# MengRao/pollnet

Hardware: AMD Instinct MI355X
Metric: device-resident Gbit/s + Mframes/s, 1500 B IPv4/TCP frames, 1/2/4/8 MI355X (higher is better)
Workload: dtype u16/u32 integer (one's-complement sums)

## Files before the change

### pollnet_amd/csrc/frame_pass.hpp

```cpp
#pragma once

#include <type_traits>

#include "device_common.hpp"

namespace pn_dev {

constexpr int kWave = 64;
constexpr int kFramesPerWave = 64;
constexpr int kBatch = 8;
constexpr int kLoadAux = 2;
constexpr int kStoreAux = 16;

constexpr int kWinChunks = 7;
constexpr int kWinBytes = 16 * kWinChunks;
using Window = Win<4 * kWinChunks>;

constexpr uint32_t kPadUnknown = 0xFFFFFFFFu;

enum : int { kAblNoProbe = 1, kAblNoReduce = 2 };
enum : int { kExactRange = 64 };
enum : int { kCoopProbe = 256 };
enum : int { kSkipEmptyLoads = 1024 };
enum : int { kSkipWaveGate = 16384 };
// ... 293 lines not shown
    }
#pragma unroll
    for (int j = 0; j < kBatch; ++j) {
      const int end = ends[j], s0 = s0s[j];
      if (end > s0 + 2048) {
        const __amdgpu_buffer_rsrc_t rs = frame_rsrc(frame_win(b0 + j), (uint32_t)(end + 15) & ~15u);
        uint32_t sum = acc[j];
        for (int kb = s0 + 2048; kb < end; kb += 1024) {
          const u32x4 w = __builtin_amdgcn_raw_buffer_load_b128(rs, kb + lane * 16, 0, LAUX);
          const int o = kb + lane * 16;
          sum = dot2(w.x, tail_sel(end, o), sum);
          sum = dot2(w.y, tail_sel(end, o + 4), sum);
          sum = dot2(w.z, tail_sel(end, o + 8), sum);
          sum = dot2(w.w, tail_sel(end, o + 12), sum);
        }
        acc[j] = sum;
      }
    }
    if constexpr (ABL & kAblNoReduce) {
      uint32_t x = 0;
#pragma unroll
      for (int j = 0; j < kBatch; ++j) x += acc[j];
      if ((uint32_t)(lane >> 3) == b0 / kBatch) t_all += x;
    } else {
#pragma unroll
      for (int i = 0; i < 4; ++i) {
        const auto r = __builtin_amdgcn_permlane32_swap(acc[i], acc[i + 4], false, false);
        acc[i] = r[0] + r[1];
      }
#pragma unroll
      for (int i = 0; i < 2; ++i) {
        const auto r = __builtin_amdgcn_permlane16_swap(acc[i], acc[i + 2], false, false);
        acc[i] = r[0] + r[1];
      }
      const bool b3 = lane & 8;
      const uint32_t keep = b3 ? acc[1] : acc[0];
      const uint32_t send = b3 ? acc[0] : acc[1];
      uint32_t v = keep + dpp<0x128>(send);
      v += dpp<0xB1>(v);
      v += dpp<0x4E>(v);
      v += dpp<0x141>(v);
      const uint32_t tot = __shfl(v, (lane & 7) * 8);
      if ((uint32_t)(lane >> 3) == b0 / kBatch) t_all += tot;
    }
  }
}

template <int ABL, int LAUX, int IDX>
__device__ __forceinline__ void stream_phase_pipelined(uint32_t stride, const uint8_t* group_ipa, uint64_t my_win,
                                                       uint32_t n_here, int lane, int end_rel, uint32_t& t_all,
                                                       uint32_t& pad) {
  static_assert(!(ABL & kSkipEmptyLoads) && (ABL & kExactRange), "pipelined phase 2: every load issued, exact ranges");
  constexpr int kHalf = kBatch / 2;
  auto frame_win = [&](uint32_t fi) -> const uint8_t* {
    if constexpr (IDX) {
      const uint32_t lo = __builtin_amdgcn_readlane((uint32_t)my_win, fi & 63);
      const uint32_t hi = __builtin_amdgcn_readlane((uint32_t)(my_win >> 32), fi & 63);
      return (const uint8_t*)(((uint64_t)hi << 32) | lo);
    } else {
      return group_ipa + (uint64_t)fi * stride;
    }
  };
  int ends[kBatch], s0s[kBatch];
  u32x4 w0s[kBatch], w1s[kBatch];
  uint32_t acc[kBatch];
  auto issue = [&](uint32_t fi0, int j0) {
#pragma unroll
    for (int q = 0; q < kHalf; ++q) {
      const int j = j0 + q;
      const uint32_t fi = fi0 + q;
      const int end = fi < n_here ? __builtin_amdgcn_readlane(end_rel, fi & 63) & ~1 : 0;
      ends[j] = end;
      const uint32_t end16 = (uint32_t)(end + 3) & ~3u;
      const uint8_t* fw = frame_win(fi);
      const int s0 = (int)stream_start((uint64_t)fw);
      s0s[j] = s0;
      const __amdgpu_buffer_rsrc_t rs = frame_rsrc(fw, end16);
      w0s[j] = __builtin_amdgcn_raw_buffer_load_b128(rs, s0 + lane * 16, 0, LAUX);
      w1s[j] = __builtin_amdgcn_raw_buffer_load_b128(rs, s0 + 1024 + lane * 16, 0, LAUX);
    }
  };
  auto consume = [&](uint32_t fi0, int j0) {
#pragma unroll
    for (int q = 0; q < kHalf; ++q) {
      const int j = j0 + q;
      const int end = ends[j], s0 = s0s[j];
      const u32x4 w0 = w0s[j], w1 = w1s[j];
      uint32_t sum = 0;
      sum = dot2(w0.x, 0x10001u, sum);
      sum = dot2(w0.y, 0x10001u, sum);
      sum = dot2(w0.z, 0x10001u, sum);
      sum = dot2(w0.w, 0x10001u, sum);
      sum = dot2(w1.x, 0x10001u, sum);
      sum = dot2(w1.y, 0x10001u, sum);
      sum = dot2(w1.z, 0x10001u, sum);
      sum = dot2(w1.w, 0x10001u, sum);
      const int q2 = end - 2 - s0;
      if ((end & 2) && q2 >= 0 && q2 < 2048) {
        const u32x4 w = (q2 < 1024) ? w0 : w1;
        const int dw = (q2 >> 2) & 3;
        const uint32_t d = dw == 0 ? w.x : dw == 1 ? w.y : dw == 2 ? w.z : w.w;
        if (lane == ((q2 & 1023) >> 4)) sum -= d >> 16;
      }
      acc[j] = sum;
      const int p = end - 1;
      if ((__builtin_amdgcn_readlane(end_rel, (fi0 + q) & 63) & 1) && p >= s0 && p < s0 + 2048) {
        const int qq = p - s0;
        const u32x4 w = (qq < 1024) ? w0 : w1;
        const int dw = (qq >> 2) & 3;
        const uint32_t d = dw == 0 ? w.x : dw == 1 ? w.y : dw == 2 ? w.z : w.w;
        const uint32_t b = __builtin_amdgcn_readlane((d >> (8 * (qq & 3))) & 0xff, (qq & 1023) >> 4);
        if ((uint32_t)lane == fi0 + q) pad = b;
      }
    }
  };
  issue(0, 0);
  for (uint32_t b0 = 0; b0 < n_here; b0 += kBatch) {
    issue(b0 + kHalf, kHalf);
    consume(b0, 0);
    issue(b0 + kBatch, 0);
    consume(b0 + kHalf, kHalf);
    if constexpr (ABL & kAblNoReduce) {
      uint32_t x = 0;
#pragma unroll
      for (int j = 0; j < kBatch; ++j) x += acc[j];
      if ((uint32_t)(lane >> 3) == b0 / kBatch) t_all += x;
      continue;
    }
    uint32_t r8[kBatch];
#pragma unroll
    for (int i = 0; i < kBatch; ++i) r8[i] = acc[i];
#pragma unroll
    for (int i = 0; i < 4; ++i) {
      const auto r = __builtin_amdgcn_permlane32_swap(r8[i], r8[i + 4], false, false);
      r8[i] = r[0] + r[1];
    }
#pragma unroll
    for (int i = 0; i < 2; ++i) {
      const auto r = __builtin_amdgcn_permlane16_swap(r8[i], r8[i + 2], false, false);
      r8[i] = r[0] + r[1];
    }
    const bool b3 = lane & 8;
    const uint32_t keep = b3 ? r8[1] : r8[0];
    const uint32_t send = b3 ? r8[0] : r8[1];
    uint32_t v = keep + dpp<0x128>(send);
    v += dpp<0xB1>(v);
    v += dpp<0x4E>(v);
    v += dpp<0x141>(v);
    const uint32_t tot = __shfl(v, (lane & 7) * 8);
    if ((uint32_t)(lane >> 3) == b0 / kBatch) t_all += tot;
  }
}

}
```

### pollnet_amd/csrc/rx_classify.hpp

```cpp
#pragma once

#include <hip/hip_runtime.h>

#include <cstdio>
#include <cstring>
#include <string>
#include <type_traits>

#include "../../include/pollnet_amd.h"
#include "device_common.hpp"
#include "frame_pass.hpp"
#include "pn_internal.hpp"

namespace {

using namespace pn_dev;
using pn_internal::g_err;
using pn_internal::hip_err;
using pn_internal::set_err;

struct KArgs {
  const uint8_t* frames;
  pn_result* out;
  const pn_conn_entry* tbl;
  uint64_t mask;
  uint32_t n_entries;
  uint32_t max_conn;
  uint32_t n;
  uint32_t stride;
  uint32_t ipa_off;
  uint32_t avail;
  const uint64_t* offs;
  uint32_t fpw = kFramesPerWave;
  uint32_t* sig_count = nullptr;
  uint32_t* sig_flag = nullptr;
  uint32_t sig_token = 0;
};

struct KArgsAux : KArgs {
  u32x4* aux = nullptr;
};

struct Probe {
  uint64_t key;
  uint32_t e;
  uint64_t k;
  uint32_t cid;
};

struct FrameState {
  uint32_t flags, ihl, tot_len, src_ip, dst_ip, seq_raw, doff, tflags, s_ip20, s_opt, tcp_len, conn_id;
  uint32_t t_all;
  int end_rel;
  uint32_t pad;
  bool trunc;
  Probe probe;
};

__device__ __forceinline__ Probe probe_issue(uint32_t src_ip, uint32_t src_port, bool live, const KArgs& a) {
  Probe p;
  const uint32_t ip_h = __builtin_bswap32(src_ip);
  const uint32_t port_h = bswap16(src_port);
  p.key = ((uint64_t)ip_h << 15) | (port_h & 0x7fff) | ((uint64_t)(port_h & 0x8000) << 32);
  p.e = (uint32_t)(p.key & a.mask);
  p.k = PN_EMPTY_KEY;
  p.cid = 0;
  if (live && p.e < a.n_entries) {
    const u32x4 ent = *reinterpret_cast<const u32x4*>(a.tbl + p.e);
    p.k = ((uint64_t)ent.y << 32) | ent.x;
    p.cid = ent.z;
  }
  return p;
}

__device__ __forceinline__ void probe_finish(const Probe& p, bool live, const KArgs& a, uint32_t& conn_id, uint32_t& flags) {
  const uint64_t key = p.key;
  uint32_t e = p.e;
  uint64_t k = p.k;
  uint32_t cid = p.cid;
  const uint32_t lane = threadIdx.x;
  bool srch = live && e < a.n_entries && k < key;
  if (__ballot(srch) != 0) {
    constexpr int kAhead = 2;
    u32x4 nx[kAhead];
#pragma unroll
    for (int j = 0; j < kAhead; ++j) {
      nx[j] = u32x4{0u, 0u, 0u, 0u};
      if (srch && e + 1 + j < a.n_entries) nx[j] = *reinterpret_cast<const u32x4*>(a.tbl + e + 1 + j);
    }
    uint32_t step = 0, cid2 = 0;
    uint64_t k2 = 0;
#pragma unroll
    for (int j = kAhead - 1; j >= 0; --j) {
      const uint64_t kk = ((uint64_t)nx[j].y << 32) | nx[j].x;
      if (e + 1 + j >= a.n_entries || kk >= key) {
        step = j + 1;
        k2 = kk;
        cid2 = nx[j].z;
      }
    }
    if (srch) {
      if (step != 0) {
        e += step;
        k = k2;
        cid = cid2;
        srch = false;
      } else {
        e += kAhead;
      }
    }
  }
  uint64_t need = __ballot(srch);
  while (need != 0) {
    const uint32_t e0 = __builtin_amdgcn_readlane(e, (uint32_t)__builtin_ctzll(need));
    uint64_t group = __ballot(srch && e == e0);
    for (uint32_t base = e0 + 1; group != 0; base += kWave) {
      const uint32_t idx = base + lane;
      u32x4 ent = {0u, 0u, 0u, 0u};
      if (idx < a.n_entries) ent = *reinterpret_cast<const u32x4*>(a.tbl + idx);
      const uint64_t kk = ((uint64_t)ent.y << 32) | ent.x;
      for (uint64_t pend = group; pend != 0; pend &= pend - 1) {
        const uint32_t L = (uint32_t)__builtin_ctzll(pend);
        const uint64_t kl = ((uint64_t)(uint32_t)__builtin_amdgcn_readlane((uint32_t)(key >> 32), L) << 32) |
                            (uint32_t)__builtin_amdgcn_readlane((uint32_t)key, L);
        const uint64_t stop = __ballot(idx >= a.n_entries || kk >= kl);
        if (stop != 0) {
          const uint32_t first = (uint32_t)__builtin_ctzll(stop);
          const uint32_t klo = __builtin_amdgcn_readlane(ent.x, first), khi = __builtin_amdgcn_readlane(ent.y, first);
          const uint32_t c = __builtin_amdgcn_readlane(ent.z, first);
          if (lane == L) {
            e = base + first;
            k = ((uint64_t)khi << 32) | klo;
            cid = c;
            srch = false;
          }
          group &= ~(1ull << L);
        }
      }
    }
    need = __ballot(srch);
  }
  if (live && e < a.n_entries && k == key) {
    conn_id = cid;
    flags |= PN_F_HIT;
    if (cid >= a.max_conn) flags |= PN_F_TW;
  }
}

template <int MIS, int ABL>
__device__ __forceinline__ FrameState header_phase(const Window& h, uint32_t ether_type, bool live, uint32_t s0,
                                                   const KArgs& a) {
  static_assert(MIS + 64 <= kWinBytes, "window must cover ip .. ip+64");
  FrameState st;
  const uint32_t ver_ihl = h.template b8<MIS + 0>();
  st.ihl = ver_ihl & 0xf;
  st.tot_len = bswap16(h.template u16<MIS + 2>());
  const uint32_t proto = h.template b8<MIS + 9>();
  st.src_ip = h.template u32<MIS + 12>();
  st.dst_ip = h.template u32<MIS + 16>();
  const uint32_t src_port = h.template u16<MIS + 20>();
  st.seq_raw = h.template u32<MIS + 24>();
  st.doff = h.template b8<MIS + 32>() >> 4;
  st.tflags = h.template b8<MIS + 33>();

  uint32_t flags = (st.tflags & 0x1f) << 4;
  if (ether_type != 0x0008 || (ver_ihl >> 4) != 4 || proto != 6) flags |= PN_F_NOT_TCP;
  if (st.ihl != 5) flags |= PN_F_IHL_NE_5;

  st.s_ip20 = h.template sum16<MIS, MIS + 20>();
  if (csum_fold(st.s_ip20) == 0) flags |= PN_F_IP_OK;
  st.s_opt = 0;
  if (st.ihl > 5) st.s_opt = h.template sum16_upto<MIS + 20, MIS + 60>(MIS + 4 * st.ihl);

  st.tcp_len = (st.tot_len - 20) & 0xffff;
  const uint32_t seg_even = (st.tcp_len + 1) & ~1u;
  st.trunc = 34 + seg_even > a.avail;
  if (st.trunc) flags |= PN_F_TRUNC;
  st.end_rel = (live && !st.trunc) ? (int)((MIS + 20 + seg_even) | (st.tcp_len & 1)) : 0;
  st.pad = kPadUnknown;

  st.t_all = window_part<MIS>(h, st.end_rel & ~1, s0);

  st.conn_id = PN_MISS;
  if constexpr (!(ABL & kAblNoProbe)) probe_finish(probe_issue(st.src_ip, src_port, live, a), live, a, st.conn_id, flags);
  st.flags = flags;
  return st;
}

template <int MIS, int ABL, int SAUX>
__device__ __forceinline__ void finish(const KArgs& a, FrameState st, uint32_t f, const uint8_t* win, bool bad_off,
                                       u32x4* lds_rec, uint32_t cx_ack = 0, uint32_t cx_wport = 0) {
  uint32_t flags = st.flags;
  uint32_t tcp_fold = 0xffff;
  if constexpr ((ABL & kHeaderOnly) != 0) {
    flags |= PN_F_TCP_UNCHECKED;
    if (!st.trunc && st.ihl >= 5 && 4 * st.ihl <= st.tot_len && csum_fold(st.s_ip20 + st.s_opt) == 0)
      flags |= PN_F_RFC_IP_OK;
  } else if (!st.trunc) {
    const uint32_t s_seg = st.t_all - st.s_ip20;
    const uint32_t s_addr = (st.src_ip >> 16) + (st.src_ip & 0xffff) + (st.dst_ip >> 16) + (st.dst_ip & 0xffff);
    tcp_fold = csum_fold(s_addr + 0x0600 + bswap16(st.tcp_len) + s_seg);
    if (tcp_fold == 0) flags |= PN_F_TCP_OK;
    const uint32_t hl = 4 * st.ihl;
    if (st.ihl >= 5 && hl <= st.tot_len) {
      if (csum_fold(st.s_ip20 + st.s_opt) == 0) flags |= PN_F_RFC_IP_OK;
      uint32_t pad = 0;
      if (st.tot_len & 1) {
        uint32_t b = st.pad;
        if (b == kPadUnknown) b = (win + MIS)[st.tot_len];
        pad = b << 8;
      }
      const uint32_t rfc = s_addr + 0x0600 + bswap16(st.tot_len - hl) + (s_seg - st.s_opt - pad);
      if (csum_fold(rfc) == 0) flags |= PN_F_RFC_TCP_OK;
    }
  }
  const int data_off = 34 + 4 * (int)st.doff;
  const int data_end = 14 + (int)min(st.tot_len, 1500u);
  u32x4 rec;
  rec.x = st.conn_id;
  rec.y = __builtin_bswap32(st.seq_raw) + ((st.tflags >> 1) & 1);
  rec.z = (uint32_t)data_off | ((uint32_t)(data_end - data_off) << 16);
  rec.w = flags | (tcp_fold << 16);
  if (bad_off) rec = u32x4{PN_MISS, 0, 0, PN_F_BADOFF};
  if constexpr (ABL & kChainAux) {
    u32x4* aux = static_cast<const KArgsAux&>(a).aux;
    if (aux) {
      aux[2 * f] = rec;
      aux[2 * f + 1] = u32x4{cx_ack, st.dst_ip, cx_wport, 0u};
    }
  }
  if (lds_rec) {
    *lds_rec = rec;
    return;
  }
  const uint32_t blk = __builtin_amdgcn_readfirstlane(f & ~63u);
  const __amdgpu_buffer_rsrc_t rs = frame_rsrc((const uint8_t*)(a.out + blk), 64 * 16);
  __builtin_amdgcn_raw_buffer_store_b128(rec, rs, (f & 63u) * 16, 0, SAUX);
}

template <int MIS, int COOP, int ABL, int LAUX, int SAUX, int IDX, int LWIN>
__device__ __forceinline__ void classify_group(const KArgs& a, const uint32_t wave_base, const int lane) {
  if (wave_base >= a.n) return;
  const uint32_t f = wave_base + lane;
  const uint32_t n_here = min(a.fpw, a.n - wave_base);
  const bool live = (uint32_t)lane < n_here;
  const uint8_t* wave_slot = a.frames + (uint64_t)wave_base * a.stride;
  const __amdgpu_buffer_rsrc_t rs = frame_rsrc(wave_slot, n_here * a.stride);

  Window h;
  uint32_t ether_type;
  const uint8_t* win = nullptr;
  bool bad_off = false;
  if constexpr (IDX) {
    const uint64_t o = live ? a.offs[f] : 0;
    bad_off = live && ((o + 14) & 15) != (uint64_t)MIS;
    win = a.frames + o + 14 - MIS;
    ether_type = load_window_indexed<MIS, COOP, LWIN>(win, o, live && !bad_off, a.avail, lane, h);
  } else {
    ether_type = load_window_strided<MIS, COOP, LWIN>(rs, lane, a.stride, a.ipa_off, (uint32_t)(uintptr_t)wave_slot, h);
  }
  if constexpr (!IDX) win = wave_slot + (uint64_t)lane * a.stride + a.ipa_off;
  FrameState st = header_phase<MIS, ABL>(h, ether_type, live && !bad_off, stream_start((uint64_t)win), a);
  if constexpr ((ABL & kHeaderOnly) != 0) {
  } else {
    const uint32_t e16 = (uint32_t)((st.end_rel & ~1) + 3) & ~3u;
    const bool short_frame = live && e16 <= stream_start((uint64_t)win) + 1024;
    constexpr int kFull = ABL & ~(kSkipEmptyLoads | kSkipWaveGate);
    if (__ballot(short_frame) == 0) {
      if constexpr (!IDX) {
        if (a.stride <= 2048)
          stream_phase_pipelined<kFull, LAUX, IDX>(a.stride, wave_slot + a.ipa_off, (uint64_t)win, n_here, lane,
                                                   st.end_rel, st.t_all, st.pad);
        else
          stream_phase<kFull, LAUX, IDX>(a.stride, wave_slot + a.ipa_off, (uint64_t)win, n_here, lane, st.end_rel,
                                         st.t_all, st.pad);
      } else {
        stream_phase<kFull, LAUX, IDX>(a.stride, wave_slot + a.ipa_off, (uint64_t)win, n_here, lane, st.end_rel,
                                       st.t_all, st.pad);
      }
    } else {
      stream_phase<ABL, LAUX, IDX>(a.stride, wave_slot + a.ipa_off, (uint64_t)win, n_here, lane, st.end_rel, st.t_all,
                                   st.pad);
    }
  }
  if constexpr (ABL & kChainAux) {
    if (live)
      finish<MIS, ABL, SAUX>(a, st, f, win, bad_off, nullptr, h.template u32<MIS + 28>(),
                             h.template u16<MIS + 22>() | (h.template u16<MIS + 34>() << 16));
  } else {
    if (live) finish<MIS, ABL, SAUX>(a, st, f, win, bad_off, nullptr);
  }
}

constexpr int kXcdOrder = 8;
constexpr int kProdGopt = (2 << 4) | kXcdOrder;
constexpr int kSignalDone = 1 << 12;
constexpr int kLiveAbl = kProdAbl | kAblNoProbe | kAblNoReduce | kHeaderOnly | kChainAux;
template <int MIS, int COOP, int ABL = kProdAbl, int LAUX = kLoadAux, int SAUX = kStoreAux, int IDX = 0, int LWIN = LAUX,
          int GRP = 1, int GOPT = kProdGopt>
__global__ __launch_bounds__(kWave, 4) void rx_classify_kernel(KArgs a) {
  static_assert(GRP == 1 && (GOPT & kXcdOrder) && !(GOPT & ~(kXcdOrder | (0xff << 4) | kSignalDone)),
                "one XCD-ordered group per workgroup: the other workgroup shapes are retired");
  static_assert((ABL & kProdAbl) == kProdAbl && !(ABL & ~kLiveAbl), "a retired form of a phase");
  const int lane = threadIdx.x;
  if constexpr (((GOPT >> 4) & 0xff) > 0) {
    __shared__ uint32_t pad_lds[((GOPT >> 4) & 0xff) * 256];
    pad_lds[lane] = lane;
    if (__builtin_amdgcn_readfirstlane(pad_lds[(lane + 1) & 63]) == 0x7fffffffu) a.n = 0;
  }
  classify_group<MIS, COOP, ABL, LAUX, SAUX, IDX, LWIN>(a, xcd_group(blockIdx.x, gridDim.x) * a.fpw, lane);
  if constexpr (GOPT & kSignalDone) signal_done(a.sig_count, a.sig_flag, a.sig_token, lane);
}


inline bool coop_layout(const KArgs& a) {
  return (a.stride % 16) == 0 && a.ipa_off >= 16 && ((uintptr_t)a.frames % 16) == 0;
}

inline void strided_kargs(KArgs& a, const void* frames, void* out, const pn_conn_entry* tbl, uint64_t mask,
                          uint32_t n_entries, uint32_t max_conn, uint32_t n, uint32_t stride, uint32_t frame_off) {
  a.frames = (const uint8_t*)frames;
  a.out = (pn_result*)out;
  a.tbl = tbl;
  a.mask = mask;
  a.n_entries = n_entries;
  a.max_conn = max_conn;
  a.n = n;
  a.stride = stride;
  a.ipa_off = (frame_off + 14) & ~15u;
  a.avail = stride - frame_off;
  a.offs = nullptr;
  a.fpw = frames_per_wave(n);
}

template <int MIS, int COOP, int ABL = kProdAbl, int LAUX = kLoadAux, int SAUX = kStoreAux, int IDX = 0, int LWIN = LAUX,
          int GOPT = kProdGopt>
void launch_one(const KArgs& a, hipStream_t s) {
  hipLaunchKernelGGL((rx_classify_kernel<MIS, COOP, ABL, LAUX, SAUX, IDX, LWIN, 1, GOPT>), dim3((a.n + a.fpw - 1) / a.fpw),
                     dim3(kWave), 0, s, a);
}

template <int MIS, bool SIG = false, bool HO = false>
void launch(const KArgs& a, hipStream_t s) {
  constexpr int G = SIG ? (kProdGopt | kSignalDone) : kProdGopt;
  constexpr int A = HO ? (kProdAbl | kHeaderOnly) : kProdAbl;
  if (coop_layout(a)) return launch_one<MIS, 1, A, kLoadAux, kStoreAux, 0, kLoadAux, G>(a, s);
  launch_one<MIS, 0, A, kLoadAux, kStoreAux, 0, kLoadAux, G>(a, s);
}
}
```

### pollnet_amd/csrc/rx_service.hip

```cpp
#include <algorithm>
#include <chrono>
#include <cstdlib>

#include "rx_classify.hpp"

namespace {
using pn_internal::hip_err;
using pn_internal::set_err;

struct alignas(64) SvcPost {
  uint32_t gen;
  uint32_t n;
  uint32_t fpw;
  uint32_t max_conn;
  const uint8_t* frames;
  pn_result* out;
  const pn_conn_entry* tbl;
  uint16_t* links;
  uint32_t mask;
  uint32_t n_entries;
  uint32_t check;
  uint32_t seq;
};
static_assert(sizeof(SvcPost) == 64, "one line per post");

constexpr uint32_t kDoneWords = 64;
constexpr uint32_t kCountWords = 64;
constexpr uint32_t kExitWord = 96;
constexpr uint32_t kWordsBytes = 512;
constexpr uint32_t kLatWaves = PN_SERVICE_WAVES;
static_assert(kLatWaves <= kDoneWords, "a latency-tier post completes through per-wave done words");
constexpr uint32_t kLatFrames = kLatWaves * kFramesPerWave;
constexpr uint32_t kNetLimitMs = 8000;
constexpr uint32_t kPostVerify = 1u << 30, kPostLinks = 1u << 29, kPostN = (1u << 21) - 1;
constexpr uint32_t kLinkFrames = PN_LINK_MAX_FRAMES, kLinkConns = PN_LINK_MAX_CONNS;
constexpr uint32_t kMailBytes = 4096;

struct alignas(64) SvcDev {
  uint32_t count[2][16];
};
constexpr uint32_t kExitFlag = 32;

#ifdef PN_SVC_TRACE
__device__ uint64_t* g_svc_trace = nullptr;
#define SVC_T(w, i)                                                       \
  do {                                                                    \
    if (lane == 0 && (w) < 64) g_svc_trace[(w) * 8 + (i)] = wall_clock64(); \
  } while (0)
#else
#define SVC_T(w, i) \
  do {              \
  } while (0)
#endif

struct SArgs {
  const SvcPost* mail;
  u32x4* scratch;
  uint32_t* done_words;
  uint32_t* exit_word;
  SvcDev* dev;
  uint64_t idle_ticks;
  uint64_t net_ticks;
  uint32_t epoch;
  uint32_t last;
  uint32_t stride, ipa_off, avail;
  uint32_t poll_sleep;
};

inline uint32_t svc_fpw(uint32_t n, bool verify) {
  uint32_t fpw = verify ? 8u : kFramesPerWave;
  while (fpw < kFramesPerWave && (n + fpw - 1) / fpw > kLatWaves) fpw <<= 1;
  return fpw;
}

inline uint32_t svc_check(const SvcPost* p, uint32_t k) {
  const uint32_t* w = reinterpret_cast<const uint32_t*>(p);
  uint32_t x = k;
  for (int i = 1; i <= 13; i++) x ^= w[i];
  return x;
}

__host__ __device__ __forceinline__ uint32_t svc_active(uint32_t n, uint32_t fpw, uint32_t waves) {
  const uint32_t groups = (n + fpw - 1) / fpw;
  return groups < waves ? groups : waves;
}

inline uint32_t svc_helpers(uint32_t n, uint32_t max) {
  if (n <= kLatFrames) return 0;
  const uint32_t groups = (n + kFramesPerWave - 1) / kFramesPerWave;
  return std::min(groups - kLatWaves, max);
}

__device__ __forceinline__ KArgsAux svc_args(uint32_t v, uint32_t b, const SArgs& s, uint32_t k) {
  auto w32 = [&](uint32_t i) { return (uint32_t)__builtin_amdgcn_readlane(v, b + i); };
  auto u64 = [&](uint32_t lo) { return ((uint64_t)w32(lo + 1) << 32) | w32(lo); };
  KArgsAux a;
  const uint32_t nw = w32(1);
  a.n = nw & kPostN;
  a.fpw = w32(2) & 0xffu;
  a.max_conn = w32(3);
  a.frames = reinterpret_cast<const uint8_t*>(u64(4));
  a.out = reinterpret_cast<pn_result*>(u64(6));
  a.tbl = reinterpret_cast<const pn_conn_entry*>(u64(8));
  a.mask = w32(12);
  a.n_entries = w32(13);
  a.stride = s.stride;
  a.ipa_off = s.ipa_off;
  a.avail = s.avail;
  a.offs = nullptr;
  a.aux = (nw & kPostLinks) ? s.scratch + (size_t)(k & 1) * kLinkFrames * 2 : nullptr;
  return a;
}

__device__ __forceinline__ uint16_t* svc_links(uint32_t v, uint32_t b) {
  return reinterpret_cast<uint16_t*>(((uint64_t)(uint32_t)__builtin_amdgcn_readlane(v, b + 11) << 32) |
                                     (uint32_t)__builtin_amdgcn_readlane(v, b + 10));
}

constexpr uint32_t kCleanNeed = PN_F_HIT | PN_F_ACK | PN_F_IP_OK;
constexpr uint32_t kCleanNone = PN_F_TW | PN_F_SYN | PN_F_FIN | PN_F_RST | PN_F_NOT_TCP | PN_F_TRUNC | PN_F_BADOFF |
                                PN_F_IHL_NE_5;

struct ChainLds {
  uint32_t last[kLinkConns];
  uint32_t key[kLinkFrames];
  uint32_t seq_end[kLinkFrames];
  u32x4 fields[kLinkFrames];
};

__device__ __forceinline__ ChainLds& chain_lds() {
  __shared__ ChainLds c;
  return c;
}

__device__ __forceinline__ void chain_init(int lane) {
  ChainLds& c = chain_lds();
  for (uint32_t i = lane; i < kLinkConns; i += kWave) c.last[i] = 0u;
  wave_lds_sync();
}

__device__ __forceinline__ void chain_step(ChainLds& c, uint32_t base, uint32_t n, uint32_t max_conn, bool on,
                                           const u32x4& rec, const u32x4& fx, const __amdgpu_buffer_rsrc_t& lr,
                                           uint64_t below, int lane) {
  const uint32_t i = base + lane;
  const bool valid = i < n;
  const uint32_t flags = rec.w & 0xffffu;
  const uint32_t len = rec.z >> 16;
  const bool member = on && valid && (flags & (PN_F_HIT | PN_F_TW)) == PN_F_HIT && rec.x < max_conn;
  const bool usable = (flags & kCleanNeed) == kCleanNeed && (flags & kCleanNone) == 0 &&
                      (flags & (PN_F_TCP_OK | PN_F_TCP_UNCHECKED)) != 0 && len != 0 && len < 0x8000u;
  const uint32_t key = member ? rec.x : 0u;
  if (valid) {
    c.key[i] = member ? key : 0xFFFFFFFFu;
    c.seq_end[i] = rec.y + len;
    c.fields[i] = u32x4{fx.x, fx.y, fx.z, (rec.z & 0xffffu) | (usable ? 0x10000u : 0u)};
  }
  uint32_t prev = 0;
  if (member) prev = c.last[key];
  wave_lds_sync();
  if (member) atomicMax(&c.last[key], i + 1);
  wave_lds_sync();
  uint64_t todo = __ballot(member && c.last[key] != i + 1);
  while (todo) {
    const uint32_t leader = (uint32_t)__builtin_ctzll(todo);
    const uint32_t kk = __builtin_amdgcn_readlane(key, leader);
    const uint64_t m = __ballot(member && key == kk);
    todo &= ~m;
    const uint64_t lower = m & below;
    if (member && key == kk && lower) prev = base + 64u - (uint32_t)__builtin_clzll(lower);
  }
  uint32_t d = 0;
  if (member && usable && prev) {
    const uint32_t j = prev - 1;
    const u32x4 pf = c.fields[j];
    if ((pf.w >> 16) && c.seq_end[j] == rec.y && pf.x == fx.x && pf.y == fx.y && pf.z == fx.z &&
        (pf.w & 0xffffu) == (rec.z & 0xffffu))
      d = i - j;
  }
  if (valid) __builtin_amdgcn_raw_buffer_store_b16((unsigned short)d, lr, i * 2, 0, 0);
  wave_lds_sync();
}

__device__ __forceinline__ void chain_pass(const u32x4* aux, uint32_t n, uint32_t max_conn, uint16_t* links, int lane) {
  constexpr int kChunk = 8;
  ChainLds& c = chain_lds();
  const bool on = max_conn <= kLinkConns;
  const __amdgpu_buffer_rsrc_t lr = frame_rsrc(reinterpret_cast<const uint8_t*>(links), n * 2);
  const __amdgpu_buffer_rsrc_t ar = frame_rsrc(reinterpret_cast<const uint8_t*>(aux), n * 32);
  const uint64_t below = (1ull << lane) - 1;
  for (uint32_t base0 = 0; base0 < n; base0 += kChunk * kWave) {
    u32x4 rec[kChunk], fx[kChunk];
#pragma unroll
    for (int s = 0; s < kChunk; ++s) {
      const uint32_t i = base0 + s * kWave + lane;
      rec[s] = __builtin_amdgcn_raw_buffer_load_b128(ar, i * 32, 0, 0);
      fx[s] = __builtin_amdgcn_raw_buffer_load_b128(ar, i * 32 + 16, 0, 0);
    }
#pragma unroll
    for (int s = 0; s < kChunk; ++s)
      if (base0 + s * kWave < n) chain_step(c, base0 + s * kWave, n, max_conn, on, rec[s], fx[s], lr, below, lane);
  }
  for (uint32_t i = lane; i < n; i += kWave) {
    const uint32_t k = c.key[i];
    if (k != 0xFFFFFFFFu) c.last[k] = 0u;
  }
  wave_lds_sync();
}

template <int MIS, int COOP, bool HELPER = false>
__device__ __forceinline__ void svc_run(const KArgsAux& a, bool verify, bool linked, uint32_t w, uint32_t act, uint32_t k,
                                        uint32_t* done_word, int lane) {
  for (uint32_t g = w; g * a.fpw < a.n; g += act) {
    if (verify) classify_group<MIS, COOP, kProdAbl | kChainAux, kLoadAux, kStoreAux, 0, kLoadAux>(a, g * a.fpw, lane);
    else
      classify_group<MIS, COOP, kProdAbl | kHeaderOnly | kChainAux, kLoadAux, kStoreAux, 0, kLoadAux>(a, g * a.fpw, lane);
  }
  if constexpr (HELPER) return;
  __threadfence_system();
  if (lane == 0 && act <= kDoneWords && !linked)
    __hip_atomic_store(done_word, k, __ATOMIC_RELAXED, __HIP_MEMORY_SCOPE_SYSTEM);
}

template <bool PASS>
__device__ __forceinline__ void svc_finish(const KArgsAux& a, uint16_t* links, uint32_t k, uint32_t* count_word, int lane) {
  if constexpr (PASS) {
    if (a.aux) {
      __builtin_amdgcn_fence(__ATOMIC_ACQUIRE, "agent");
      chain_pass(a.aux, a.n, a.max_conn, links, lane);
    }
  }
  __threadfence_system();
  if (lane == 0) __hip_atomic_store(count_word, k, __ATOMIC_RELAXED, __HIP_MEMORY_SCOPE_SYSTEM);
}

template <bool PASS>
__device__ __forceinline__ void svc_count(uint32_t* count, const KArgsAux& a, uint16_t* links, uint32_t target, uint32_t k,
                                          uint32_t* count_word, int lane) {
  uint32_t prev = 0;
  if (lane == 0) prev = atomicAdd(count, 1u);
  prev = __builtin_amdgcn_readfirstlane(prev);
  if (prev == target - 1) {
    if (lane == 0) __hip_atomic_store(count, 0u, __ATOMIC_RELAXED, __HIP_MEMORY_SCOPE_AGENT);
    svc_finish<PASS>(a, links, k, count_word, lane);
  }
}

template <int MIS, int COOP>
__global__ __launch_bounds__(kWave) void rx_service_kernel(SArgs s) {
  const int lane = threadIdx.x;
  const uint32_t w = blockIdx.x, W = gridDim.x;
  const uint32_t* mw = reinterpret_cast<const uint32_t*>(s.mail);
  uint32_t last = s.last;
  uint64_t t0 = wall_clock64();
  chain_init(lane);
  for (;;) {
    const uint32_t v = lane <= (int)kExitFlag ? __hip_atomic_load(mw + lane, __ATOMIC_RELAXED, __HIP_MEMORY_SCOPE_SYSTEM) : 0u;
    if (w != 0 && (uint32_t)__builtin_amdgcn_readlane(v, kExitFlag) == s.epoch) return;
    const uint32_t k = last + 1;
    const uint32_t b = (k & 1) * 16;
    const uint32_t q = __builtin_amdgcn_readlane(v, b + 15);
    uint32_t x = q;
#pragma unroll
    for (uint32_t i = 1; i <= 13; i++) x ^= (uint32_t)__builtin_amdgcn_readlane(v, b + i);
    const bool whole = (uint32_t)__builtin_amdgcn_readlane(v, b) == q && (uint32_t)__builtin_amdgcn_readlane(v, b + 14) == x;
    if (!whole || (int32_t)(q - k) < 0) {
      if (w == 0) {
        if (wall_clock64() - t0 > s.idle_ticks) {
          if (lane == 0) {
            __hip_atomic_store(const_cast<uint32_t*>(mw) + kExitFlag, s.epoch, __ATOMIC_RELAXED, __HIP_MEMORY_SCOPE_SYSTEM);
            __hip_atomic_store(s.exit_word, s.epoch, __ATOMIC_RELEASE, __HIP_MEMORY_SCOPE_SYSTEM);
          }
          return;
        }
        __builtin_amdgcn_s_sleep(1);
      } else {
        if (wall_clock64() - t0 > s.net_ticks) return;
        for (uint32_t i = 0; i < s.poll_sleep; ++i) __builtin_amdgcn_s_sleep(1);
      }
      continue;
    }
    if (q != k) {
      last = k;
      t0 = wall_clock64();
      continue;
    }
    const uint32_t nw = __builtin_amdgcn_readlane(v, b + 1);
    if (nw == PN_SERVICE_STOP) return;
    last = k;
    const uint32_t fw = __builtin_amdgcn_readlane(v, b + 2);
    const uint32_t act = svc_active(nw & kPostN, fw & 0xffu, W + (fw >> 8));
    if (w < act) {
      SVC_T(w, 0);
      __builtin_amdgcn_fence(__ATOMIC_ACQUIRE, "");
      SVC_T(w, 1);
      const KArgsAux a = svc_args(v, b, s, k);
      SVC_T(w, 5);
      const bool linked = a.aux != nullptr;
      svc_run<MIS, COOP>(a, (nw & kPostVerify) != 0, linked, w, act, k, s.done_words + w, lane);
      SVC_T(w, 6);
      if (act > kDoneWords || linked) {
        uint32_t* cw = s.done_words + kCountWords + (k & 1);
        if (act == 1) svc_finish<true>(a, svc_links(v, b), k, cw, lane);
        else svc_count<true>(&s.dev->count[k & 1][0], a, svc_links(v, b), act < W ? act : W, k, cw, lane);
      }
      SVC_T(w, 7);
    }
    t0 = wall_clock64();
  }
}

template <int MIS, int COOP>
__global__ __launch_bounds__(kWave) void rx_service_helper_kernel(KArgsAux a, uint32_t verify, uint32_t act) {
  svc_run<MIS, COOP, true>(a, verify != 0, false, kLatWaves + blockIdx.x, act, 0, nullptr, threadIdx.x);
}

template <int MIS>
void launch_svc(bool coop, uint32_t waves, const SArgs& a, hipStream_t s) {
  if (coop) hipLaunchKernelGGL((rx_service_kernel<MIS, 1>), dim3(waves), dim3(kWave), 0, s, a);
  else hipLaunchKernelGGL((rx_service_kernel<MIS, 0>), dim3(waves), dim3(kWave), 0, s, a);
}

template <int MIS>
void launch_helpers(bool coop, uint32_t helpers, const KArgsAux& a, uint32_t verify, uint32_t act, hipStream_t s) {
  if (coop) hipLaunchKernelGGL((rx_service_helper_kernel<MIS, 1>), dim3(helpers), dim3(kWave), 0, s, a, verify, act);
  else hipLaunchKernelGGL((rx_service_helper_kernel<MIS, 0>), dim3(helpers), dim3(kWave), 0, s, a, verify, act);
}
}

struct pn_service {
  pn_ctx* ctx = nullptr;
  hipStream_t stream = nullptr;
  hipStream_t helper_stream = nullptr;
  uint32_t stride = 0, frame_off = 0;
  uint32_t helpers_max = 0;
  uint32_t post_helpers[2] = {0, 0};
  hipEvent_t helper_ev[2] = {nullptr, nullptr};
  uint64_t idle_ticks = 0, net_ticks = 0;
  SvcPost* mail = nullptr;
  bool mail_dev = false;
  uint32_t* words = nullptr;
  uint32_t post_words[2] = {0, 0};
  uint32_t tbl_post[2] = {0, 0};
  bool tbl_used[2] = {false, false};
  SvcDev* dev = nullptr;
  u32x4* scratch = nullptr;
  uint32_t seq = 0;
  uint32_t epoch = 0;
  bool running = false;
  bool coop = false;
};

namespace {
SArgs svc_sargs(const pn_service* v, uint32_t base) {
  SArgs a;
  a.mail = v->mail;
  a.scratch = v->scratch;
  a.done_words = v->words;
  a.exit_word = v->words + kExitWord;
  a.dev = v->dev;
  a.idle_ticks = v->idle_ticks;
  a.net_ticks = v->net_ticks;
  a.epoch = v->epoch;
  a.last = base;
  a.stride = v->stride;
  a.ipa_off = (v->frame_off + 14) & ~15u;
  a.avail = v->stride - v->frame_off;
  a.poll_sleep = v->mail_dev ? 1u : 16u;
  return a;
}

inline void host_sfence() { asm volatile("sfence" ::: "memory"); }

void svc_publish(SvcPost* slot, const SvcPost& q, bool wc) {
  static const bool avx = __builtin_cpu_supports("avx");
  if (wc && avx) {
    asm volatile(
        "vmovdqu (%0), %%ymm0\n\t"
        "vmovdqu 32(%0), %%ymm1\n\t"
        "vmovntdq %%ymm0, (%1)\n\t"
        "vmovntdq %%ymm1, 32(%1)\n\t"
        "sfence\n\t"
// ... 281 lines not shown
```

Baseline: 53080.

## Add contiguous-span checksum path using wave prefix scan for densely packed indexed frames

For indexed frames, the code now checks whether a wave's frames are densely packed and non-overlapping in one region. If they are, it streams the whole span with coalesced 16-byte buffer loads, double-buffered in blocks of 8 per lane. Per-chunk sums go into LDS, and a wave-wide inclusive prefix scan over the cells lets each lane take its frame's sum as a difference of prefix values. This replaces per-frame strided loads with fully coalesced reads, at the cost of LDS syncs, scan work and a density check on every wave.

```diff
diff --git a/pollnet_amd/csrc/frame_pass.hpp b/pollnet_amd/csrc/frame_pass.hpp
--- a/pollnet_amd/csrc/frame_pass.hpp
+++ b/pollnet_amd/csrc/frame_pass.hpp
@@ -469,4 +469,87 @@
   }
 }
 
-}
+constexpr int kContigBlk = 8;
+constexpr int kContigCells = 64 * kContigBlk;
+
+__device__ __forceinline__ uint32_t wave_scan_incl(uint32_t v) {
+  v += (uint32_t)__builtin_amdgcn_update_dpp(0, (int)v, 0x111, 0xf, 0xf, false);
+  v += (uint32_t)__builtin_amdgcn_update_dpp(0, (int)v, 0x112, 0xf, 0xf, false);
+  v += (uint32_t)__builtin_amdgcn_update_dpp(0, (int)v, 0x114, 0xf, 0xf, false);
+  v += (uint32_t)__builtin_amdgcn_update_dpp(0, (int)v, 0x118, 0xf, 0xf, false);
+  v += (uint32_t)__builtin_amdgcn_update_dpp(0, (int)v, 0x142, 0xa, 0xf, false);
+  v += (uint32_t)__builtin_amdgcn_update_dpp(0, (int)v, 0x143, 0xc, 0xf, false);
+  return v;
+}
+
+template <int LAUX>
+__device__ __forceinline__ void stream_phase_contig(const uint8_t* base, uint32_t span, uint32_t nch, int relw, int s0,
+                                                    int end, bool odd, int lane, uint32_t& t_all, uint32_t& pad) {
+  uint32_t* cells = reinterpret_cast<uint32_t*>(coop_tile());
+  const __amdgpu_buffer_rsrc_t rs = frame_rsrc(base, (span + 3) & ~3u);
+  const bool has = end > s0;
+  const int tail_lo = (end - 1) & ~15;
+  const int ca = has ? (relw + s0) >> 4 : 0, cb = has ? (relw + tail_lo) >> 4 : 0;
+  const u32x4 tw = __builtin_amdgcn_raw_buffer_load_b128(rs, has ? (uint32_t)(relw + tail_lo) : kNoFetch, 0, 0);
+  u32x4 wa[kContigBlk], wb[kContigBlk];
+  auto issue = [&](u32x4(&w)[kContigBlk], uint32_t k) {
+#pragma unroll
+    for (int j = 0; j < kContigBlk; ++j)
+      w[j] = __builtin_amdgcn_raw_buffer_load_b128(rs, (k * kContigCells + 64 * j + lane) * 16, 0, LAUX);
+  };
+  uint32_t carry = 0, sum = 0;
+  auto consume = [&](const u32x4(&w)[kContigBlk], uint32_t k) {
+    wave_lds_sync();
+#pragma unroll
+    for (int j = 0; j < kContigBlk; ++j) {
+      uint32_t c = dot2(w[j].x, 0x10001u, 0);
+      c = dot2(w[j].y, 0x10001u, c);
+      c = dot2(w[j].z, 0x10001u, c);
+      c = dot2(w[j].w, 0x10001u, c);
+      cells[64 * j + lane] = c;
+    }
+    wave_lds_sync();
+    u32x4* row = reinterpret_cast<u32x4*>(cells) + 2 * lane;
+    u32x4 q0 = row[0], q1 = row[1];
+    q0.y += q0.x;
+    q0.z += q0.y;
+    q0.w += q0.z;
+    q1.x += q0.w;
+    q1.y += q1.x;
+    q1.z += q1.y;
+    q1.w += q1.z;
+    const uint32_t incl = wave_scan_incl(q1.w);
+    const uint32_t ex = incl - q1.w + carry;
+    row[0] = u32x4{q0.x + ex, q0.y + ex, q0.z + ex, q0.w + ex};
+    row[1] = u32x4{q1.x + ex, q1.y + ex, q1.z + ex, q1.w + ex};
+    wave_lds_sync();
+    const int kb = (int)(k * kContigCells);
+    const int lo = min(max(ca - kb, 0), kContigCells), hi = min(max(cb - kb, 0), kContigCells);
+    const uint32_t vlo = cells[max(lo, 1) - 1], vhi = cells[max(hi, 1) - 1];
+    sum += (hi ? vhi : carry) - (lo ? vlo : carry);
+    carry += __builtin_amdgcn_readlane(incl, 63);
+  };
+  const uint32_t nblk = (nch + kContigCells - 1) / kContigCells;
+  issue(wa, 0);
+  for (uint32_t k = 0; k < nblk; k += 2) {
+    issue(wb, k + 1);
+    consume(wa, k);
+    issue(wa, k + 2);
+    consume(wb, k + 1);
+  }
+  if (has) {
+    const int nb = end - tail_lo;
+    sum = dot2(tw.x, tail_sel(nb, 0), sum);
+    sum = dot2(tw.y, tail_sel(nb, 4), sum);
+    sum = dot2(tw.z, tail_sel(nb, 8), sum);
+    sum = dot2(tw.w, tail_sel(nb, 12), sum);
+    if (odd) {
+      const int q = nb - 1, dw = q >> 2;
+      const uint32_t d = dw == 0 ? tw.x : dw == 1 ? tw.y : dw == 2 ? tw.z : tw.w;
+      pad = (d >> (8 * (q & 3))) & 0xff;
+    }
+  }
+  t_all += sum;
+}
+
+}
diff --git a/pollnet_amd/csrc/rx_classify.hpp b/pollnet_amd/csrc/rx_classify.hpp
--- a/pollnet_amd/csrc/rx_classify.hpp
+++ b/pollnet_amd/csrc/rx_classify.hpp
@@ -266,7 +266,36 @@
     const uint32_t e16 = (uint32_t)((st.end_rel & ~1) + 3) & ~3u;
     const bool short_frame = live && e16 <= stream_start((uint64_t)win) + 1024;
     constexpr int kFull = ABL & ~(kSkipEmptyLoads | kSkipWaveGate);
-    if (__ballot(short_frame) == 0) {
+    bool dense = false;
+    uint32_t d = 0, s0_first = 0;
+    uint64_t win_first = 0;
+    if constexpr (IDX && !(ABL & kAblNoReduce)) {
+      const uint64_t w = (uint64_t)win;
+      win_first = ((uint64_t)(uint32_t)__builtin_amdgcn_readfirstlane((uint32_t)(w >> 32)) << 32) |
+                  (uint32_t)__builtin_amdgcn_readfirstlane((uint32_t)w);
+      const uint32_t s0 = stream_start(w), end = (uint32_t)(st.end_rel & ~1);
+      s0_first = __builtin_amdgcn_readfirstlane(s0);
+      const uint64_t d64 = w - win_first;
+      d = (uint32_t)d64;
+      const uint32_t d_next = (uint32_t)__builtin_amdgcn_update_dpp((int)d, (int)d, 0x130, 0xf, 0xf, false);
+      const uint32_t start_next = (uint32_t)__builtin_amdgcn_update_dpp((int)(d + s0), (int)(d + s0), 0x130, 0xf, 0xf, false);
+      bool ok = !bad_off && !st.trunc && d64 < (1u << 18) && end <= s0 + 2048 && d + end < s0_first + (128u << 10);
+      if ((uint32_t)lane + 1 < n_here) ok = ok && d_next > d && d_next - d <= a.avail && d + end <= start_next;
+      dense = __all(!live || ok);
+    }
+    if (dense) {
+      if constexpr (IDX) {
+        const int s0 = (int)stream_start((uint64_t)win), end = st.end_rel & ~1, relw = (int)d - (int)s0_first;
+        const uint64_t streams = __ballot(end > s0);
+        if (streams != 0) {
+          const uint32_t last = 63u - (uint32_t)__builtin_clzll(streams);
+          const uint32_t span = __builtin_amdgcn_readlane(relw + end, last);
+          const uint32_t nch = __builtin_amdgcn_readlane((relw + ((end - 1) & ~15)) >> 4, last);
+          stream_phase_contig<LAUX>((const uint8_t*)(win_first + s0_first), span, nch, relw, s0, end, st.end_rel & 1, lane,
+                                    st.t_all, st.pad);
+        }
+      }
+    } else if (__ballot(short_frame) == 0) {
       if constexpr (!IDX) {
         if (a.stride <= 2048)
           stream_phase_pipelined<kFull, LAUX, IDX>(a.stride, wave_slot + a.ipa_off, (uint64_t)win, n_here, lane,
```

Result: slower. 51870 (-2.3%).

## Precompute intra-wave chain links during classify and shrink serial chain pass

Applied to the files above, without the earlier changes.

Moves most of the per-connection chain-linking work into the parallel classify phase. Each wave finds, within itself, the nearest earlier frame on the same connection and checks continuity with shuffles, then writes a chain word into the aux record. The single-wave chain pass now only resolves links that cross wave boundaries. It does this with a 16-bit last-index table in LDS, all records loaded up front into registers, and batched gathers of predecessor records. This cuts the LDS traffic and serial per-step work of the finishing pass, but adds LDS sync and shuffle work to every classify wave and raises register pressure in chain_pass. Timing trace macros are added under the existing trace flag.

```diff
diff --git a/pollnet_amd/csrc/rx_classify.hpp b/pollnet_amd/csrc/rx_classify.hpp
--- a/pollnet_amd/csrc/rx_classify.hpp
+++ b/pollnet_amd/csrc/rx_classify.hpp
@@ -40,6 +40,53 @@
 struct KArgsAux : KArgs {
   u32x4* aux = nullptr;
 };
+
+constexpr uint32_t kCleanNeed = PN_F_HIT | PN_F_ACK | PN_F_IP_OK;
+constexpr uint32_t kCleanNone = PN_F_TW | PN_F_SYN | PN_F_FIN | PN_F_RST | PN_F_NOT_TCP | PN_F_TRUNC | PN_F_BADOFF |
+                                PN_F_IHL_NE_5;
+
+__device__ __forceinline__ bool chain_usable(uint32_t flags, uint32_t len) {
+  return (flags & kCleanNeed) == kCleanNeed && (flags & kCleanNone) == 0 &&
+         (flags & (PN_F_TCP_OK | PN_F_TCP_UNCHECKED)) != 0 && len != 0 && len < 0x8000u;
+}
+
+constexpr uint32_t kChainNear = 0x7fu, kChainTail = 0x100u, kChainCont = 0x200u, kChainMember = 0x400u;
+
+__device__ __forceinline__ u32x4 chain_entry(const u32x4& rec, uint32_t ack, uint32_t dst_ip, uint32_t wport, bool live,
+                                             uint32_t max_conn, int lane) {
+  __shared__ uint8_t owner[256];
+  const uint32_t conn_id = rec.x, flags = rec.w & 0xffffu, len = rec.z >> 16;
+  const bool member = live && (flags & (PN_F_HIT | PN_F_TW)) == PN_F_HIT && conn_id < max_conn;
+  if (member) owner[conn_id & 255u] = (uint8_t)lane;
+  wave_lds_sync();
+  uint64_t todo = __ballot(member && owner[conn_id & 255u] != (uint8_t)lane);
+  uint32_t near = 0;
+  bool tail = member;
+  const bool repeats = todo != 0;
+  while (todo) {
+    const uint32_t kk = __builtin_amdgcn_readlane(conn_id, (uint32_t)__builtin_ctzll(todo));
+    const bool mine = member && conn_id == kk;
+    const uint64_t m = __ballot(mine);
+    todo &= ~m;
+    if (mine) {
+      const uint64_t lower = m & ((1ull << lane) - 1);
+      if (lower) near = (uint32_t)lane - (63u - (uint32_t)__builtin_clzll(lower));
+      tail = (m >> lane) == 1ull;
+    }
+  }
+  wave_lds_sync();
+  uint32_t word = member ? kChainMember | near | (tail ? kChainTail : 0u) : 0u;
+  if (repeats) {
+    const bool usable = chain_usable(flags, len);
+    const uint32_t own_w = (rec.z & 0xffffu) | (usable ? 0x10000u : 0u);
+    const int src = (lane - (int)near) & 63;
+    const uint32_t p_end = __shfl(rec.y + len, src), p_ack = __shfl(ack, src), p_ip = __shfl(dst_ip, src);
+    const uint32_t p_wp = __shfl(wport, src), p_w = __shfl(own_w, src);
+    if (near != 0 && usable && p_w == own_w && p_end == rec.y && p_ack == ack && p_ip == dst_ip && p_wp == wport)
+      word |= kChainCont;
+  }
+  return u32x4{ack, dst_ip, wport, word};
+}
 
 struct Probe {
   uint64_t key;
@@ -189,7 +236,7 @@
 
 template <int MIS, int ABL, int SAUX>
 __device__ __forceinline__ void finish(const KArgs& a, FrameState st, uint32_t f, const uint8_t* win, bool bad_off,
-                                       u32x4* lds_rec, uint32_t cx_ack = 0, uint32_t cx_wport = 0) {
+                                       u32x4* lds_rec, u32x4* rec_out = nullptr) {
   uint32_t flags = st.flags;
   uint32_t tcp_fold = 0xffff;
   if constexpr ((ABL & kHeaderOnly) != 0) {
@@ -222,13 +269,7 @@
   rec.z = (uint32_t)data_off | ((uint32_t)(data_end - data_off) << 16);
   rec.w = flags | (tcp_fold << 16);
   if (bad_off) rec = u32x4{PN_MISS, 0, 0, PN_F_BADOFF};
-  if constexpr (ABL & kChainAux) {
-    u32x4* aux = static_cast<const KArgsAux&>(a).aux;
-    if (aux) {
-      aux[2 * f] = rec;
-      aux[2 * f + 1] = u32x4{cx_ack, st.dst_ip, cx_wport, 0u};
-    }
-  }
+  if constexpr (ABL & kChainAux) *rec_out = rec;
   if (lds_rec) {
     *lds_rec = rec;
     return;
@@ -284,9 +325,16 @@
     }
   }
   if constexpr (ABL & kChainAux) {
-    if (live)
-      finish<MIS, ABL, SAUX>(a, st, f, win, bad_off, nullptr, h.template u32<MIS + 28>(),
-                             h.template u16<MIS + 22>() | (h.template u16<MIS + 34>() << 16));
+    u32x4 rec = {PN_MISS, 0u, 0u, 0u};
+    if (live) finish<MIS, ABL, SAUX>(a, st, f, win, bad_off, nullptr, &rec);
+    if (u32x4* aux = static_cast<const KArgsAux&>(a).aux) {
+      const u32x4 cx = chain_entry(rec, h.template u32<MIS + 28>(), st.dst_ip,
+                                   h.template u16<MIS + 22>() | (h.template u16<MIS + 34>() << 16), live, a.max_conn, lane);
+      if (live) {
+        aux[2 * f] = rec;
+        aux[2 * f + 1] = cx;
+      }
+    }
   } else {
     if (live) finish<MIS, ABL, SAUX>(a, st, f, win, bad_off, nullptr);
   }
diff --git a/pollnet_amd/csrc/rx_service.hip b/pollnet_amd/csrc/rx_service.hip
--- a/pollnet_amd/csrc/rx_service.hip
+++ b/pollnet_amd/csrc/rx_service.hip
@@ -47,9 +47,27 @@
   do {                                                                    \
     if (lane == 0 && (w) < 64) g_svc_trace[(w) * 8 + (i)] = wall_clock64(); \
   } while (0)
+#define SVC_CLK(v) const uint64_t v = wall_clock64()
+#define SVC_PUT(w, i, v)                                        \
+  do {                                                          \
+    if (lane == 0 && (w) < 64) g_svc_trace[(w) * 8 + (i)] = (v); \
+  } while (0)
+#define SVC_PASS(j, v)                             \
+  do {                                             \
+    if (lane == 0) g_svc_trace[512 + (j)] = (v); \
+  } while (0)
 #else
 #define SVC_T(w, i) \
   do {              \
+  } while (0)
+#define SVC_CLK(v) \
+  do {             \
+  } while (0)
+#define SVC_PUT(w, i, v) \
+  do {                   \
+  } while (0)
+#define SVC_PASS(j, v) \
+  do {                 \
   } while (0)
 #endif
 
@@ -117,15 +135,11 @@
                                      (uint32_t)__builtin_amdgcn_readlane(v, b + 10));
 }
 
-constexpr uint32_t kCleanNeed = PN_F_HIT | PN_F_ACK | PN_F_IP_OK;
-constexpr uint32_t kCleanNone = PN_F_TW | PN_F_SYN | PN_F_FIN | PN_F_RST | PN_F_NOT_TCP | PN_F_TRUNC | PN_F_BADOFF |
-                                PN_F_IHL_NE_5;
+constexpr int kChainSteps = kLinkFrames / kWave;
+static_assert(kLinkFrames % kWave == 0 && kLinkFrames < 65536, "whole steps; 1 + a frame's index in 16 bits");
 
 struct ChainLds {
-  uint32_t last[kLinkConns];
-  uint32_t key[kLinkFrames];
-  uint32_t seq_end[kLinkFrames];
-  u32x4 fields[kLinkFrames];
+  uint16_t last[kLinkConns];
 };
 
 __device__ __forceinline__ ChainLds& chain_lds() {
@@ -134,77 +148,99 @@
 }
 
 __device__ __forceinline__ void chain_init(int lane) {
-  ChainLds& c = chain_lds();
-  for (uint32_t i = lane; i < kLinkConns; i += kWave) c.last[i] = 0u;
+  uint32_t* w = reinterpret_cast<uint32_t*>(chain_lds().last);
+  for (uint32_t i = lane; i < kLinkConns / 2; i += kWave) w[i] = 0u;
   wave_lds_sync();
 }
 
-__device__ __forceinline__ void chain_step(ChainLds& c, uint32_t base, uint32_t n, uint32_t max_conn, bool on,
-                                           const u32x4& rec, const u32x4& fx, const __amdgpu_buffer_rsrc_t& lr,
-                                           uint64_t below, int lane) {
-  const uint32_t i = base + lane;
-  const bool valid = i < n;
-  const uint32_t flags = rec.w & 0xffffu;
-  const uint32_t len = rec.z >> 16;
-  const bool member = on && valid && (flags & (PN_F_HIT | PN_F_TW)) == PN_F_HIT && rec.x < max_conn;
-  const bool usable = (flags & kCleanNeed) == kCleanNeed && (flags & kCleanNone) == 0 &&
-                      (flags & (PN_F_TCP_OK | PN_F_TCP_UNCHECKED)) != 0 && len != 0 && len < 0x8000u;
-  const uint32_t key = member ? rec.x : 0u;
-  if (valid) {
-    c.key[i] = member ? key : 0xFFFFFFFFu;
-    c.seq_end[i] = rec.y + len;
-    c.fields[i] = u32x4{fx.x, fx.y, fx.z, (rec.z & 0xffffu) | (usable ? 0x10000u : 0u)};
-  }
-  uint32_t prev = 0;
-  if (member) prev = c.last[key];
-  wave_lds_sync();
-  if (member) atomicMax(&c.last[key], i + 1);
-  wave_lds_sync();
-  uint64_t todo = __ballot(member && c.last[key] != i + 1);
-  while (todo) {
-    const uint32_t leader = (uint32_t)__builtin_ctzll(todo);
-    const uint32_t kk = __builtin_amdgcn_readlane(key, leader);
-    const uint64_t m = __ballot(member && key == kk);
-    todo &= ~m;
-    const uint64_t lower = m & below;
-    if (member && key == kk && lower) prev = base + 64u - (uint32_t)__builtin_clzll(lower);
-  }
-  uint32_t d = 0;
-  if (member && usable && prev) {
-    const uint32_t j = prev - 1;
-    const u32x4 pf = c.fields[j];
-    if ((pf.w >> 16) && c.seq_end[j] == rec.y && pf.x == fx.x && pf.y == fx.y && pf.z == fx.z &&
-        (pf.w & 0xffffu) == (rec.z & 0xffffu))
-      d = i - j;
-  }
-  if (valid) __builtin_amdgcn_raw_buffer_store_b16((unsigned short)d, lr, i * 2, 0, 0);
-  wave_lds_sync();
-}
-
-__device__ __forceinline__ void chain_pass(const u32x4* aux, uint32_t n, uint32_t max_conn, uint16_t* links, int lane) {
-  constexpr int kChunk = 8;
+__device__ __forceinline__ void chain_pass(const u32x4* aux, uint32_t n, uint32_t max_conn, uint32_t fpw, uint16_t* links,
+                                           int lane) {
+  constexpr int kGather = 8;
+  static_assert(kChainSteps % kGather == 0, "whole gather rounds");
   ChainLds& c = chain_lds();
   const bool on = max_conn <= kLinkConns;
+  const bool multi = fpw < kWave;
   const __amdgpu_buffer_rsrc_t lr = frame_rsrc(reinterpret_cast<const uint8_t*>(links), n * 2);
   const __amdgpu_buffer_rsrc_t ar = frame_rsrc(reinterpret_cast<const uint8_t*>(aux), n * 32);
   const uint64_t below = (1ull << lane) - 1;
-  for (uint32_t base0 = 0; base0 < n; base0 += kChunk * kWave) {
-    u32x4 rec[kChunk], fx[kChunk];
-#pragma unroll
-    for (int s = 0; s < kChunk; ++s) {
-      const uint32_t i = base0 + s * kWave + lane;
-      rec[s] = __builtin_amdgcn_raw_buffer_load_b128(ar, i * 32, 0, 0);
-      fx[s] = __builtin_amdgcn_raw_buffer_load_b128(ar, i * 32 + 16, 0, 0);
-    }
-#pragma unroll
-    for (int s = 0; s < kChunk; ++s)
-      if (base0 + s * kWave < n) chain_step(c, base0 + s * kWave, n, max_conn, on, rec[s], fx[s], lr, below, lane);
-  }
-  for (uint32_t i = lane; i < n; i += kWave) {
-    const uint32_t k = c.key[i];
-    if (k != 0xFFFFFFFFu) c.last[k] = 0u;
-  }
+  SVC_CLK(t_in);
+  u32x4 rec[kChainSteps], fx[kChainSteps];
+#pragma unroll
+  for (int s = 0; s < kChainSteps; ++s) {
+    const uint32_t i = s * kWave + lane;
+    rec[s] = __builtin_amdgcn_raw_buffer_load_b128(ar, i * 32, 0, 0);
+    fx[s] = __builtin_amdgcn_raw_buffer_load_b128(ar, i * 32 + 16, 0, 0);
+  }
+#pragma unroll
+  for (int s = 0; s < kChainSteps; ++s)
+    if (!on) fx[s].w = 0u;
+  SVC_CLK(t_loaded);
+  uint32_t prev[kChainSteps];
+#pragma unroll
+  for (int s = 0; s < kChainSteps; ++s) {
+    prev[s] = 0;
+    if (s * kWave < n) {
+      const uint32_t i = s * kWave + lane, key = rec[s].x;
+      const bool head = (fx[s].w & (kChainMember | kChainNear)) == kChainMember, tail = (fx[s].w & kChainTail) != 0;
+      if (head) prev[s] = c.last[key];
+      wave_lds_sync();
+      if (tail) c.last[key] = (uint16_t)(i + 1);
+      wave_lds_sync();
+      if (multi) {
+        uint64_t todo = __ballot(tail && c.last[key] != (uint16_t)(i + 1));
+        while (todo) {
+          const uint32_t kk = __builtin_amdgcn_readlane(key, (uint32_t)__builtin_ctzll(todo));
+          const uint64_t mt = __ballot(tail && key == kk);
+          todo &= ~mt;
+          const uint64_t lower = mt & below;
+          if (head && key == kk && lower) prev[s] = s * kWave + 64u - (uint32_t)__builtin_clzll(lower);
+          if (lane == 63 - (int)__builtin_clzll(mt)) c.last[key] = (uint16_t)(i + 1);
+        }
+        wave_lds_sync();
+      }
+    }
+  }
+  SVC_CLK(t_walked);
+#pragma unroll
+  for (int s = 0; s < kChainSteps; ++s)
+    if (s * kWave < n && (fx[s].w & kChainTail)) c.last[rec[s].x] = 0;
   wave_lds_sync();
+  SVC_CLK(t_reset);
+#pragma unroll
+  for (int h = 0; h < kChainSteps / kGather; ++h) {
+    if (h * kGather * kWave >= n) break;
+    u32x4 prec[kGather], pfx[kGather];
+#pragma unroll
+    for (int g = 0; g < kGather; ++g) {
+      const uint32_t off = prev[h * kGather + g] ? (prev[h * kGather + g] - 1) * 32 : kNoFetch;
+      prec[g] = __builtin_amdgcn_raw_buffer_load_b128(ar, off, 0, 0);
+      pfx[g] = __builtin_amdgcn_raw_buffer_load_b128(ar, off + 16, 0, 0);
+    }
+#pragma unroll
+    for (int g = 0; g < kGather; ++g) {
+      const int s = h * kGather + g;
+      if (s * kWave >= n) break;
+      const u32x4 r = rec[s], f = fx[s];
+      uint32_t link = (f.w & kChainCont) ? f.w & kChainNear : 0u;
+      if (__ballot(prev[s] != 0)) {
+        const u32x4 q = prec[g];
+        const bool usable = chain_usable(r.w & 0xffffu, r.z >> 16) && chain_usable(q.w & 0xffffu, q.z >> 16);
+        if (prev[s] != 0 && usable && (q.z & 0xffffu) == (r.z & 0xffffu) && q.y + (q.z >> 16) == r.y && pfx[g].x == f.x &&
+            pfx[g].y == f.y && pfx[g].z == f.z)
+          link = s * kWave + lane + 1 - prev[s];
+      }
+      prev[s] = link;
+    }
+  }
+  SVC_CLK(t_linked);
+#pragma unroll
+  for (int s = 0; s < kChainSteps; ++s)
+    if (s * kWave < n) __builtin_amdgcn_raw_buffer_store_b16((unsigned short)prev[s], lr, (s * kWave + lane) * 2, 0, 0);
+  SVC_PASS(0, t_in);
+  SVC_PASS(1, t_loaded);
+  SVC_PASS(2, t_walked);
+  SVC_PASS(3, t_reset);
+  SVC_PASS(4, t_linked);
 }
 
 template <int MIS, int COOP, bool HELPER = false>
@@ -225,8 +261,11 @@
 __device__ __forceinline__ void svc_finish(const KArgsAux& a, uint16_t* links, uint32_t k, uint32_t* count_word, int lane) {
   if constexpr (PASS) {
     if (a.aux) {
+      SVC_CLK(t_pass);
       __builtin_amdgcn_fence(__ATOMIC_ACQUIRE, "agent");
-      chain_pass(a.aux, a.n, a.max_conn, links, lane);
+      chain_pass(a.aux, a.n, a.max_conn, a.fpw, links, lane);
+      SVC_PUT(blockIdx.x, 2, t_pass);
+      SVC_T(blockIdx.x, 3);
     }
   }
   __threadfence_system();
```

Result: no change. 50980 before, 50990 after, median of 4 (+0.0%).
